# razoumov/radiativeTransfer

Measured on AMD Instinct MI355X. Metric: cell·dir·ν updates/sec per iteration, 256³ grid; achieved HBM GB/s vs peak, higher is better.
Workload: dtype f64

## Files before the change

radiativetransfer_amd/csrc/ftte_api.cpp:

```cpp
#include "ftte_context.h"

using namespace ftte;

namespace ftte {

std::string g_create_error;

int fail(ftte_ctx *c, int code, const std::string &msg)
{
    if (c) c->err = msg;
    else g_create_error = msg;
    return code;
}

int fold_status(int rc)
{
    return rc == 1 ? FTTE_ERR_PHI : rc == 2 ? FTTE_ERR_THETA : FTTE_ERR_DOMINANT_AXIS;
}

}


extern "C" {

// ... 33 lines not shown
    (void)hipSetDevice(c->device);
    if (c->stream) (void)hipStreamSynchronize(c->stream);
    for (int l = 0; l < 3; ++l) {
        if (c->kappa[l]) (void)hipFree(c->kappa[l]);
        if (c->kappa_tiled[l]) (void)hipFree(c->kappa_tiled[l]);
        if (c->emis[l]) (void)hipFree(c->emis[l]);
        for (int s = 0; s < kMaxAcc; ++s) if (c->acc[l][s]) (void)hipFree(c->acc[l][s]);
    }
    if (c->d_bdeps) (void)hipFree(c->d_bdeps);
    if (c->d_bdone) (void)hipFree(c->d_bdone);
    if (c->d_bqueue) (void)hipFree(c->d_bqueue);
    if (c->d_bsync) (void)hipFree(c->d_bsync);
    if (c->h_berror) (void)hipHostFree(c->h_berror);
    if (c->d_blayers) (void)hipFree(c->d_blayers);
    if (c->d_bgroups) (void)hipFree(c->d_bgroups);
    if (c->d_btasks) (void)hipFree(c->d_btasks);
    if (c->d_faces) (void)hipFree(c->d_faces);
    if (c->d_layers) (void)hipFree(c->d_layers);
    if (c->d_items) (void)hipFree(c->d_items);
    if (c->d_uvb) (void)hipFree(c->d_uvb);
    free_forests(c);
    free_hybrid(c);
    if (c->d_leaf_of_base) (void)hipFree(c->d_leaf_of_base);
    for (int l = 0; l < 3; ++l) if (c->base_kappa[l]) (void)hipFree(c->base_kappa[l]);
    for (int l = 0; l < 3; ++l) if (c->base_emis[l]) (void)hipFree(c->base_emis[l]);
    for (int l = 0; l < 3; ++l) {
        if (c->fine_kappa[l]) (void)hipFree(c->fine_kappa[l]);
        if (c->fine_emis[l]) (void)hipFree(c->fine_emis[l]);
        for (int a = 0; a < kMaxAcc; ++a) if (c->fine_acc[l][a]) (void)hipFree(c->fine_acc[l][a]);
    }
    if (c->amr_Iout) (void)hipFree(c->amr_Iout);
    if (c->amr_mean) (void)hipFree(c->amr_mean);
    if (c->d_amr_dirs) (void)hipFree(c->d_amr_dirs);
    if (c->d_amr_tables) (void)hipFree(c->d_amr_tables);
    if (c->amr_kappa) (void)hipFree(c->amr_kappa);
    if (c->amr_emis) (void)hipFree(c->amr_emis);
    if (c->merge_stream) (void)hipStreamDestroy(c->merge_stream);
    if (c->ev_layout_done) (void)hipEventDestroy(c->ev_layout_done);
    if (c->ev_merge_done) (void)hipEventDestroy(c->ev_merge_done);
    if (c->ev_layouts_ready) (void)hipEventDestroy(c->ev_layouts_ready);
    if (c->ev_sweep_done) (void)hipEventDestroy(c->ev_sweep_done);
    for (auto &q : c->lane_stream) (void)hipStreamDestroy(q);
    for (auto &e : c->pipe_up) (void)hipEventDestroy(e);
    for (auto &e : c->lane_done) (void)hipEventDestroy(e);
    if (c->ev_fork) (void)hipEventDestroy(c->ev_fork);
    for (auto &e : c->ev_combine) if (e) (void)hipEventDestroy(e);
    if (c->host_J_dev) (void)hipFree(c->host_J_dev);
    for (int q = 0; q < 2; ++q) {
        if (c->stage[q]) (void)hipHostFree(c->stage[q]);
        if (c->stage_ev[q]) (void)hipEventDestroy(c->stage_ev[q]);
    }
    for (auto &r : c->registered) (void)hipHostUnregister((void *)r.base);
    c->point.release();
    c->drop_chem_grid();
    if (c->chem_k) (void)hipFree(c->chem_k);
    if (c->chem_counters) (void)hipFree(c->chem_counters);
    if (c->chem_mass) (void)hipFree(c->chem_mass);
    for (auto &t : c->timing) {
        (void)hipEventDestroy(t.start); (void)hipEventDestroy(t.stop);
// ... 77 lines not shown
    if ((rc = upload(c, c->kappa[0], kappa, sizeof(double) * nnu * c->ncell))) return rc;
    c->nnu = nnu;
    c->kappa_ready[0] = true; c->kappa_ready[1] = c->kappa_ready[2] = c->kappa_ready[3] = false;
    ++c->n_kappa_sets;
    return FTTE_OK;
}

int ftte_set_opacity_device(ftte_ctx *c, int nnu, const double *kappa_dev)
{
    int rc = check_ready(c, false);
    if (rc) return rc;
    if (nnu < 1 || !kappa_dev) return fail(c, FTTE_ERR_ARG, "ftte_set_opacity_device: bad argument");
    FTTE_HIP(c, hipSetDevice(c->device));
    if ((rc = wait_sweep(c))) return rc;
    if ((rc = ensure_kappa(c, nnu))) return rc;
    const bool all_three = !c->use_forest && c->kappa[1] && c->kappa[2] && c->kappa_ready[1] && c->kappa_ready[2] && c->nnu == nnu && !c->tiled_opt;
    if (all_three) {
        if (launch_set_layouts(kappa_dev, c->kappa[0], c->kappa[1], c->kappa[2], c->n, nnu, (long)c->ncell, c->stream))
            return fail(c, FTTE_ERR_NO_DEVICE, "layout kernel launch failed");
    } else FTTE_HIP(c, hipMemcpyAsync(c->kappa[0], kappa_dev, sizeof(double) * nnu * c->ncell, hipMemcpyDeviceToDevice, c->stream));
    FTTE_HIP(c, hipStreamSynchronize(c->stream));
    c->nnu = nnu;
    c->kappa_ready[0] = true; c->kappa_ready[1] = c->kappa_ready[2] = all_three; c->kappa_ready[3] = false;
    ++c->n_kappa_sets;
    return FTTE_OK;
}

int ftte_set_species(ftte_ctx *c, int nnu, const double *HI, const double *HeI, const double *HeII, const double *beta)
{
    int rc = check_ready(c, false);
    if (rc) return rc;
    if (nnu < 1 || !HI || !HeI || !HeII || !beta) return fail(c, FTTE_ERR_ARG, "ftte_set_species: bad argument");
    FTTE_HIP(c, hipSetDevice(c->device));
    if ((rc = wait_sweep(c))) return rc;
    FTTE_HIP(c, hipStreamSynchronize(c->stream));
    if ((rc = ensure_kappa(c, nnu))) return rc;
    double *tmp = nullptr;
    const size_t nc = (size_t)c->ncell;
// ... 97 lines not shown
    } else if (!std::strcmp(key, "atomic_acc")) {
        if (value < 0 || value > 1) return fail(c, FTTE_ERR_ARG, "atomic_acc must be 0 or 1");
        c->atomic_acc = value;
    } else if (!std::strcmp(key, "ablate")) {
        if (value < 0 || value > 63) return fail(c, FTTE_ERR_ARG, "ablate is a mask of 6 bits");
        c->ablate = value;
    } else if (!std::strcmp(key, "forest_fuse")) {
        if (value < 0 || value > (1 << 24)) return fail(c, FTTE_ERR_ARG, "forest_fuse must be 0 (a launch per level) .. 16777216");
        c->forest_fuse = value;
    } else if (!std::strcmp(key, "queue_mix")) {
        if (value < 0 || value > 2) return fail(c, FTTE_ERR_ARG, "queue_mix must be 0, 1 or 2");
        c->queue_mix = value;
    } else if (!std::strcmp(key, "dataflow")) {
        if (value < 0 || value > 3) return fail(c, FTTE_ERR_ARG, "dataflow must be 0 (a launch per stage), 1 (one launch, bricks wait for each other), 2 (the same with write-through stores) or 3 (persistent workgroups, a task queue per XCD)");
        c->dataflow = value;
    } else if (!std::strcmp(key, "lanes")) {
        if (value < 1 || value > 16) return fail(c, FTTE_ERR_ARG, "lanes (streams the brick sweep spreads its frequency groups over) must be 1..16");
        c->lanes = value;
    } else if (!std::strcmp(key, "team")) {
        if (value < -1 || value > 2 || value == 1) return fail(c, FTTE_ERR_ARG, "team must be -1 (by the number of frequency groups: 2 up to four, else 0), 0 (one wavefront sweeps a group's directions in turn) or 2 (two wavefronts per brick, four rows each); 1 (a wavefront per direction) lost everywhere and is gone");
        c->team = value;
    } else if (!std::strcmp(key, "tiled")) {
        if (value < 0 || value > 2) return fail(c, FTTE_ERR_ARG, "tiled must be 0 (default), 1 (bricks: opacities and accumulators stored brick by brick where the grid is made of whole bricks: a brick's layer in one piece) or 2 (the whole brick in one piece)");
        c->tiled_opt = value;
    } else if (!std::strcmp(key, "pair_waves")) {
        if (value < 2 || value > 4) return fail(c, FTTE_ERR_ARG, "pair_waves (workgroups of two wavefronts per SIMD the pair kernel is built for) must be 2..4");
        c->pair_waves = value;
    } else if (!std::strcmp(key, "share")) {
        if (value < 0 || value > 2) return fail(c, FTTE_ERR_ARG, "share (groups sharing a J accumulator) must be 0 (none), 1 (passes of one izone) or 2 (and izone pairs)");
        c->share = value;
// ... 113 lines not shown
    if (!std::strcmp(name, "grid_builds")) return c->n_grid_builds;
    if (!std::strcmp(name, "plan_builds")) return c->n_plan_builds;
    if (!std::strcmp(name, "forest_builds")) return c->n_forest_builds;
    if (!std::strcmp(name, "hybrid_boxes")) return (c->hplan.valid && c->hplan.worthwhile) ? c->hplan.most_boxes : 0;
    if (!std::strcmp(name, "hybrid_passes")) return (c->hplan.valid && c->hplan.worthwhile) ? c->hplan.npass : 0;
    if (!std::strcmp(name, "fine_block")) return (c->hplan.valid && c->hplan.worthwhile && c->hplan.fine.active) ? c->hplan.fine.n : 0;
    if (!std::strcmp(name, "brick_form")) return c->last_brick_form;
    if (!std::strcmp(name, "brick_dataflow")) return c->last_brick_dataflow;
    if (!std::strcmp(name, "brick_chunk")) return c->bplan.valid ? c->bplan.chunk : 0;
    if (!std::strcmp(name, "brick_queue_mix")) return (c->bplan.valid && c->bplan.persistent) ? c->bplan.qmix : -1;
    if (!std::strcmp(name, "brick_groups")) return c->bplan.valid ? (long long)c->bplan.groups.size() : 0;
    if (!std::strcmp(name, "brick_accumulators")) return c->bplan.valid ? c->bplan.nacc[0] + c->bplan.nacc[1] + c->bplan.nacc[2] : 0;
    if (!std::strcmp(name, "brick_accumulators_0")) return c->bplan.valid ? c->bplan.nacc[0] : 0;
    if (!std::strcmp(name, "brick_accumulators_1")) return c->bplan.valid ? c->bplan.nacc[1] : 0;
    if (!std::strcmp(name, "brick_accumulators_2")) return c->bplan.valid ? c->bplan.nacc[2] : 0;
    return -1;
}

int ftte_launch_count(const ftte_ctx *c) { return !c ? 0 : c->multi ? multi_first(c)->timing_used : c->timing_used; }

int ftte_launch_info(ftte_ctx *c, int idx, double *ms, int64_t *updates)
{
    if (c && c->multi) return ftte_launch_info(multi_first(c), idx, ms, updates);
    if (!c || idx < 0 || idx >= c->timing_used) return FTTE_ERR_ARG;
    float t = 0.f;
    const LaunchTiming &T = c->timing[idx];
    if (T.lanes > 0) {
        float begin = 0.f, end = 0.f;
        for (int l = 0; l < T.lanes; ++l) {
            float b = 0.f, e = 0.f;
// ... 571 lines not shown
```

radiativetransfer_amd/csrc/ftte_context.h:

```cpp
#pragma once

#include <hip/hip_runtime_api.h>

#include <algorithm>
#include <cmath>
#include <cstdio>
#include <cstring>
#include <functional>
#include <string>
#include <vector>

#include <thread>

#include "../../include/ftte.h"
#include "ftte_amr.h"
#include "ftte_geometry.h"
#include "ftte_internal.h"
#include "ftte_kernels.h"
#include "ftte_point.h"


namespace ftte {


// ... 46 lines not shown
    std::vector<int32_t> deps;
    bool persistent = false;
    int qnnu = 0, nq = 0, qmix = 0;
    std::vector<uint32_t> queue;
    uint32_t qoff[kBrickQueues] = {}, qlen[kBrickQueues] = {};
    int64_t qload[kBrickQueues] = {};
    int ut = kBrickRows, uw = 0;
    int64_t uqface_off = 0;
    int nslot = 2;
    int glanes = 1, nstages = 0;
    std::vector<size_t> stage_off;
    int64_t updates = 0;
    int ntu = 0, ntv = 0, nti = 0, up = 0, vp = 0, max_dirs = 0;
    int64_t face_elems = 0, vface_off = 0, iface_off = 0;
    int nacc[3] = {0, 0, 0};
};

struct LaunchTiming {
    hipEvent_t start = nullptr, stop = nullptr;
    int64_t updates = 0;
    std::vector<hipEvent_t> first, last;
    int lanes = 0;
};


}

using namespace ftte;


// ... 74 lines not shown
        uint8_t *active = nullptr;
        std::vector<int64_t> depth_off;
        double w = 0;
    };
    std::vector<ForestDev> forests;
    std::vector<double> forest_key;
    AmrDirRec *d_amr_dirs = nullptr; size_t d_amr_dirs_cap = 0;
    int64_t *d_amr_tables = nullptr; size_t d_amr_tables_cap = 0;
    double *amr_Iout = nullptr, *amr_mean = nullptr;
    double *amr_kappa = nullptr, *amr_emis = nullptr;
    size_t amr_kappa_cap = 0, amr_emis_cap = 0;
    size_t amr_scratch_cap = 0;

    hipStream_t merge_stream = nullptr;
    hipEvent_t ev_layout_done = nullptr, ev_merge_done = nullptr, ev_layouts_ready = nullptr;
    hipEvent_t ev_sweep_done = nullptr;
    bool sweep_pending = false;

    int hybrid = 1;
    int hybrid_slots = 1;
    int use_graph = 0;
    int forest_batch = 0;
    int hybrid_lanes = 1;
    int halves = 3;
    static constexpr int kMaxPipes = 4;
    hipEvent_t ev_combine[kMaxPipes] = {nullptr, nullptr, nullptr, nullptr};
    struct HybridPlan {
        bool valid = false, worthwhile = false;
        std::vector<double> key;
        BrickPlan bricks;
// ... 188 lines not shown
```

radiativetransfer_amd/csrc/ftte_internal.h:

```cpp
#pragma once
#include <cstdint>

#include "ftte_math.h"

namespace ftte {

enum RayClass : int {
    RC_ONE = 0,
    RC_TWO_U = 1,
    RC_TWO_V = 2,
    RC_THREE_U = 3,
    RC_THREE_V = 4,
    RC_THREE_U_SWAP = 5,
    RC_THREE_V_SWAP = 6
};

struct LayerRec {
    double dpath[3];
    int32_t info;
    int32_t drift;
};
static_assert(sizeof(LayerRec) == 32, "LayerRec must be 32 bytes");

struct DirRec {
// ... 6 lines not shown
    int32_t u_lo, v_lo;
    int32_t first;
    double w;
};

struct WorkItem {
    int16_t slot;
    int16_t tu, tv;
    int16_t i_first, i_last;
    int16_t pad;
};
static_assert(sizeof(WorkItem) == 12, "WorkItem must be 12 bytes");

constexpr int kMaxSlots = 16;
constexpr int kMaxAcc = 32;

struct LaunchRec {
    DirRec dir[kMaxSlots];
    const WorkItem *items;
    const double *uvb;
    int64_t group_stride;
    int32_t n;
    int32_t nitems;
    int32_t nnu;
    int32_t emit;
    ftte_consts math;
};

constexpr int kBrickRows = 8;
constexpr int kBrickDeps = 6;
// ... 169 lines not shown
```

radiativetransfer_amd/csrc/ftte_kernels.h:

```cpp
#pragma once
#include <hip/hip_runtime_api.h>

#include "ftte_internal.h"

namespace ftte {

void set_lds_pad(int bytes);
int lds_pad();
int launch_sweep(const LaunchRec &L, int rows, int waves, int stack, int nnu, hipStream_t stream);
int launch_brick(const BrickLaunch &L, int max_dirs, int waves, hipStream_t stream, bool masked = false, int persistent = 0);
int launch_xcc_census(unsigned *mask_dev, hipStream_t stream);
int launch_brick_pair(const BrickLaunch &L, int max_dirs, int waves, hipStream_t stream);
int launch_to_layout(int layout, const double *src, double *dst, int n, int nnu, long group_stride, hipStream_t stream, bool tiled = false, int tchunk = 0);
int launch_set_layouts(const double *src, double *dst0, double *dst1, double *dst2, int n, int nnu, long group_stride, hipStream_t stream);
int launch_merge(const double *const *acc, const int *layout, int count, double *J, int n, int nnu, long group_stride,
                 bool accumulate, hipStream_t stream, const int32_t *leaf_of_base = nullptr, long j_stride = 0, bool tiled = false, int tchunk = 0);
int launch_sum_parts(const double *const *parts, int nparts, double *out, long count, hipStream_t stream);
int launch_base_cells(const double *leaf_values, const int32_t *leaf_of_base, double *base_values, long nbase, long ncell, int nnu,
                      hipStream_t stream);
int launch_amr_export(const AmrLevelRec &A, int64_t most_exports, hipStream_t stream);
int launch_amr_fine_import(const AmrLevelRec &A, int64_t most_imports, hipStream_t stream);
int launch_opacity(const double *HI, const double *HeI, const double *HeII, const double *beta, double *kappa, long ncell,
                   int nnu, hipStream_t stream);

int launch_cell_major(const double *src, double *dst, long ncell, int nnu, hipStream_t stream, const int32_t *cells = nullptr, long count = 0);
int launch_amr_level(const AmrLevelRec &A, hipStream_t stream);
int launch_amr_levels(const AmrLevelRec &A, const int64_t *tables, int ndepth, hipStream_t stream);
int launch_amr_combine(const AmrLevelRec &A, double *J, bool zero_first, hipStream_t stream);

int launch_rate_table(const FreqBin *bins, int nbins, double *tables, double *logtab, hipStream_t stream);
int launch_rate_lookup(const double *logtab, int dust, int nsample, const double *tau, double *out, hipStream_t stream);
// ... 16 lines not shown
```

radiativetransfer_amd/csrc/ftte_kernels.hip:

```cpp
#include <hip/hip_runtime.h>

#include "ftte_internal.h"
#include "ftte_kernels.h"
#include "ftte_math.h"

namespace ftte {

using gcbyte = const __attribute__((address_space(1))) char;
using gbyte = __attribute__((address_space(1))) char;
using gcdouble = const __attribute__((address_space(1))) double;
using gdouble = __attribute__((address_space(1))) double;

__device__ __forceinline__ double from_lane_below(double x)
{
    int lo = __double2loint(x), hi = __double2hiint(x);
    lo = __builtin_amdgcn_update_dpp(lo, lo, 0x138, 0xf, 0xf, false);
    hi = __builtin_amdgcn_update_dpp(hi, hi, 0x138, 0xf, 0xf, false);
    return __hiloint2double(hi, lo);
}

__device__ __forceinline__ int clampi(int x, int lo, int hi) { return x < lo ? lo : (x > hi ? hi : x); }

__device__ __forceinline__ int uniform(int x) { return __builtin_amdgcn_readfirstlane(x); }
__device__ __forceinline__ long uniform(long x)
// ... 331 lines not shown

__global__ void __launch_bounds__(256) set_layouts_kernel(const double *__restrict__ src, double *__restrict__ dst0, double *__restrict__ dst1,
                                                          double *__restrict__ dst2, int n, long group_stride)
{
    __shared__ double tile[32][33];
    const long g = blockIdx.z / n;
    const int ic = blockIdx.z % n;
    const int j0 = blockIdx.y * 32, k0 = blockIdx.x * 32;
    const int tx = threadIdx.x & 31, ty = threadIdx.x >> 5;
    const long base = g * group_stride;
    for (int r = ty; r < 32; r += 8)
        if (j0 + r < n && k0 + tx < n) {
            const double v = src[base + ((long)ic * n + j0 + r) * n + k0 + tx];
            tile[r][tx] = v;
            dst0[base + ((long)ic * n + j0 + r) * n + k0 + tx] = v;
            dst1[base + ((long)(j0 + r) * n + ic) * n + k0 + tx] = v;
        }
    __syncthreads();
    for (int r = ty; r < 32; r += 8)
        if (k0 + r < n && j0 + tx < n) dst2[base + ((long)(k0 + r) * n + ic) * n + j0 + tx] = tile[tx][r];
}

int launch_set_layouts(const double *src, double *dst0, double *dst1, double *dst2, int n, int nnu, long group_stride, hipStream_t stream)
{
    const dim3 grid((n + 31) / 32, (n + 31) / 32, n * nnu);
    hipLaunchKernelGGL(set_layouts_kernel, grid, dim3(256), 0, stream, src, dst0, dst1, dst2, n, group_stride);
    return hipGetLastError() == hipSuccess ? 0 : -2;
}

int launch_to_layout(int layout, const double *src, double *dst, int n, int nnu, long group_stride, hipStream_t stream, bool tiled, int tchunk)
{
// ... 6 lines not shown
        const dim3 grid((n + 31) / 32, (n + 31) / 32, n * nnu);
        if (tiled) hipLaunchKernelGGL(to_layout2_kernel<true>, grid, dim3(256), 0, stream, src, dst, n, group_stride, tchunk);
        else hipLaunchKernelGGL(to_layout2_kernel<false>, grid, dim3(256), 0, stream, src, dst, n, group_stride, tchunk);
    } else return -1;
    return hipGetLastError() == hipSuccess ? 0 : -2;
}

struct MergeRec {
    const double *acc[3 * kMaxAcc];
    int layout[3 * kMaxAcc];
    int count;
};

template <bool tiled>
__global__ void __launch_bounds__(256) merge_kernel(const MergeRec M, double *__restrict__ J, int n, long group_stride, int accumulate,
                                                    const int32_t *__restrict__ leaf_of_base, long j_stride, int tchunk)
{
    __shared__ double tile[32][33];
    const long g = blockIdx.z / n;
    const int ic = blockIdx.z % n;
    const int j0 = blockIdx.y * 32, k0 = blockIdx.x * 32;
    const int tx = threadIdx.x & 31, ty = threadIdx.x >> 5;
    double sum[4] = {0.0, 0.0, 0.0, 0.0};
    bool have = false;
    if (accumulate && !leaf_of_base) {
        for (int q = 0; q < 4; ++q) {
            const int jc = j0 + ty + 8 * q, kc = k0 + tx;
            if (jc < n && kc < n) sum[q] = __builtin_nontemporal_load(&J[g * group_stride + ((long)ic * n + jc) * n + kc]);
        }
        have = true;
    }
    int a0 = 0;
    while (a0 < M.count && M.layout[a0] != 2) {
        int nb = 0;
        while (nb < 8 && a0 + nb < M.count && M.layout[a0 + nb] != 2) ++nb;
        double v[8][4];
// ... 51 lines not shown
        else if (leaf_of_base[b] >= 0) {
            double *dst = &J[g * j_stride + leaf_of_base[b]];
            *dst = accumulate ? *dst + sum[q] : sum[q];
        }
    }
}

int launch_merge(const double *const *acc, const int *layout, int count, double *J, int n, int nnu, long group_stride,
                 bool accumulate, hipStream_t stream, const int32_t *leaf_of_base, long j_stride, bool tiled, int tchunk)
{
    if (count > 3 * kMaxAcc) return -1;
    MergeRec M;
    M.count = count;
    for (int a = 0; a < count; ++a) { M.acc[a] = acc[a]; M.layout[a] = layout[a]; }
    const dim3 grid((n + 31) / 32, (n + 31) / 32, n * nnu);
    if (tiled) hipLaunchKernelGGL(merge_kernel<true>, grid, dim3(256), 0, stream, M, J, n, group_stride, accumulate ? 1 : 0, leaf_of_base, j_stride, tchunk);
    else hipLaunchKernelGGL(merge_kernel<false>, grid, dim3(256), 0, stream, M, J, n, group_stride, accumulate ? 1 : 0, leaf_of_base, j_stride, tchunk);
    return hipGetLastError() == hipSuccess ? 0 : -2;
}

__device__ __forceinline__ void amr_segment(const AmrLevelRec &A, const AmrDirRec &D, int64_t begin, unsigned e, unsigned nu, unsigned nnu)
{
    const SegRec R = D.rec[begin + e];
    const int seg = R.seg, up = R.up, up2 = R.up2;
    const size_t at = (size_t)(unsigned)seg * nnu + nu;
    double I;
    if (up == -3) I = D.faces[(size_t)nu * A.face_stride + (size_t)R.at];
    else if (up < 0) I = A.uvb[nu];
    else {
        I = D.Iout[(size_t)(unsigned)up * nnu + nu];
        if (up2 >= 0) I = 0.5 * (I + D.Iout[(size_t)(unsigned)up2 * nnu + nu]);
    }
// ... 945 lines not shown
```

radiativetransfer_amd/csrc/ftte_plan.cpp:

```cpp
#include "ftte_context.h"

namespace ftte {

int plan_direction(ftte_ctx *c, int d, double phi_d, double theta_d, double w_d, int tile_rows, std::vector<ftte_pattern> &pat,
                   std::vector<int> &du_cum, std::vector<int> &dv_cum, DirPlan &D, LayerRec *layers_of_d, size_t layer_off,
                   const SubGridPlan *sub)
{
    const int n = sub ? sub->n : c->n;
    const double cell = sub ? sub->cell : c->box / (double)n;
    const long nn = (long)n * n;
    D.w = w_d;

    int rc = fold_direction(phi_d, theta_d, &D.phi, &D.theta, &D.izone);
    if (rc) {
        char buf[160];
        std::snprintf(buf, sizeof buf, "direction %d (phi=%.17g, theta=%.17g) cannot be folded: %s", d, phi_d, theta_d,
                      rc == 1 ? "phi on a quadrant boundary" : rc == 2 ? "theta outside (-pi/2,0)u(0,pi/2)"
                                                                       : "tie between dominant axes");
        return fail(c, fold_status(rc), buf);
    }
    if (sub) {
        const int src = sub->patterns(d, D.phi, D.theta, D.izone, pat.data());
        if (src) return fail(c, src, "direction " + std::to_string(d) + ": ray pattern left the unit cell (sub-layer patterns of a refined block)");
    } else if (layer_patterns(n, D.phi, D.theta, pat.data())) {
// ... 355 lines not shown
            auto &V = visits[(size_t)G.layout * kMaxAcc + G.acc];
            if (V.empty()) V.resize(nb);
            const DirPlan &D0 = P.dirs[G.dirs[0]];
            const int bu = D0.su < 0 ? P.ntu - 1 - T.tu : T.tu, bv = D0.sv < 0 ? P.ntv - 1 - T.tv : T.tv, bi = D0.si < 0 ? P.nti - 1 - ti : ti;
            V[((size_t)bi * P.ntv + bv) * P.ntu + bu].push_back({T.tu + T.tv + ti + G.offset, (int32_t)q});
        }
        for (auto &V : visits)
            for (auto &list : V) {
                std::sort(list.begin(), list.end(), [](const Visit &x, const Visit &y) { return x.launch < y.launch; });
                for (size_t k = 1; k < list.size(); ++k) P.deps[(size_t)list[k].task * kBrickDeps + 3] = list[k - 1].task;
            }
        for (size_t q = 0; q < nt; ++q)
            for (int k = 0; k < kBrickDeps; ++k)
                if (P.deps[q * kBrickDeps + k] >= (int32_t)q) return fail(c, FTTE_ERR_STATE, "brick plan: a dependency does not precede its brick");
    }
    P.persistent = false;
    if (P.dataflow && want_dataflow == 3 && !P.tasks.empty()) {
        const int nq = c->xcc_count;
        P.persistent = true; P.qnnu = nnu; P.nq = nq; P.qmix = c->queue_mix;
        std::vector<int64_t> acc_dirs(3 * (size_t)kMaxAcc, 0);
        for (const auto &G : P.groups) acc_dirs[(size_t)G.layout * kMaxAcc + G.acc] += (int64_t)G.dirs.size();
        std::vector<int> queue_of((size_t)nnu * 3 * kMaxAcc, -1);
        int64_t load[kBrickQueues] = {};
        if (nnu % nq == 0 && c->queue_mix == 0) {
            for (int nu = 0; nu < nnu; ++nu)
                for (size_t a = 0; a < acc_dirs.size(); ++a)
                    if (acc_dirs[a]) { queue_of[(size_t)nu * acc_dirs.size() + a] = nu % nq; load[nu % nq] += acc_dirs[a]; }
        } else if (c->queue_mix == 2) {
            for (int nu = 0; nu < nnu; ++nu) {
                int k = 0;
// ... 38 lines not shown
```

radiativetransfer_amd/csrc/ftte_sweeps.cpp:

```cpp
#include <cstdlib>

#include "ftte_context.h"

namespace ftte {

int ensure_kappa(ftte_ctx *c, int nnu)
{
    const size_t need = (size_t)nnu * c->ncell;
    if (c->kappa[0] && c->kappa_cap >= need) return FTTE_OK;
    for (int l = 0; l < 3; ++l) {
        if (c->kappa[l]) { FTTE_HIP(c, hipFree(c->kappa[l])); c->kappa[l] = nullptr; }
        if (c->kappa_tiled[l]) { FTTE_HIP(c, hipFree(c->kappa_tiled[l])); c->kappa_tiled[l] = nullptr; }
        if (c->emis[l]) { FTTE_HIP(c, hipFree(c->emis[l])); c->emis[l] = nullptr; }
    }
    c->emit_mode = 0;
    FTTE_HIP(c, hipMalloc((void **)&c->kappa[0], need * sizeof(double)));
    c->kappa_cap = need;
    return FTTE_OK;
}

int check_ready(ftte_ctx *c, bool need_kappa)
{
    if (c && c->multi)
        return fail(c, FTTE_ERR_UNSUPPORTED, "a multi-device context (ftte_create with ndev > 1) takes host arrays through ftte_set_grid, ftte_set_opacity, "
// ... 397 lines not shown
        c->acc_cap = per_acc;
    }
    const size_t face_need = (size_t)ndir * nnu * (size_t)P.face_elems;
    if ((rc = ensure(c, &c->d_faces, &c->d_faces_cap, face_need))) return rc;
    if (!c->merge_stream) {
        FTTE_HIP(c, hipStreamCreateWithFlags(&c->merge_stream, hipStreamNonBlocking));
        FTTE_HIP(c, hipEventCreateWithFlags(&c->ev_layout_done, hipEventDisableTiming));
        FTTE_HIP(c, hipEventCreateWithFlags(&c->ev_merge_done, hipEventDisableTiming));
        FTTE_HIP(c, hipEventCreateWithFlags(&c->ev_layouts_ready, hipEventDisableTiming));
    }
    const bool lane_ends = pipe != nullptr;
    bool lane_layout[3] = {false, false, false};
    const bool tiled = c->tiled_opt && !pipe && !c->emit_mode && n % 64 == 0 && n % kBrickRows == 0 &&
                       (c->tiled_opt == 1 || n % P.chunk == 0);
    const int tchunk = tiled && c->tiled_opt == 2 ? P.chunk : 0;
    for (int l = 0; l < 3; ++l) {
        for (int s = 0; s < P.nacc[l]; ++s)
            if (!c->acc[l][s]) FTTE_HIP(c, hipMalloc((void **)&c->acc[l][s], sizeof(double) * c->acc_cap));
        if (P.nacc[l] && tiled) {
            if (c->kappa_tiled_from[l] != c->n_kappa_sets || c->kappa_tiled_chunk[l] != tchunk) {
                if (!c->kappa_tiled[l]) FTTE_HIP(c, hipMalloc((void **)&c->kappa_tiled[l], sizeof(double) * c->kappa_cap));
                if (launch_to_layout(l, c->kappa[0], c->kappa_tiled[l], n, nnu, (long)c->ncell, stream, true, tchunk))
                    return fail(c, FTTE_ERR_NO_DEVICE, "layout kernel launch failed");
                c->kappa_tiled_from[l] = c->n_kappa_sets;
                c->kappa_tiled_chunk[l] = tchunk;
            }
        } else if (P.nacc[l] && !c->kappa_ready[l]) {
            if (!c->kappa[l]) FTTE_HIP(c, hipMalloc((void **)&c->kappa[l], sizeof(double) * c->kappa_cap));
            if (!lane_ends) {
                if (launch_to_layout(l, c->kappa[0], c->kappa[l], n, nnu, (long)c->ncell, stream))
                    return fail(c, FTTE_ERR_NO_DEVICE, "layout kernel launch failed");
                c->kappa_ready[l] = true;
            } else lane_layout[l] = true;
        }
        if (P.nacc[l] && c->emit_mode && !c->emis_ready[l]) {
            if (!c->emis[l]) FTTE_HIP(c, hipMalloc((void **)&c->emis[l], sizeof(double) * c->kappa_cap));
            if (launch_to_layout(l, c->emis[0], c->emis[l], n, nnu, (long)c->ncell, stream))
                return fail(c, FTTE_ERR_NO_DEVICE, "layout kernel launch failed");
            c->emis_ready[l] = true;
        }
    }

    if (!c->bplan_uploaded) {
        c->bgroups_sent.clear();
        if ((rc = ensure(c, &c->d_blayers, &c->d_blayers_cap, P.layers.size()))) return rc;
        if ((rc = ensure(c, &c->d_btasks, &c->d_btasks_cap, P.tasks.size()))) return rc;
        if ((rc = ensure(c, &c->d_bgroups, &c->d_bgroups_cap, P.groups.size()))) return rc;
        if (!P.layers.empty())
            FTTE_HIP(c, hipMemcpy(c->d_blayers, P.layers.data(), sizeof(LayerRec) * P.layers.size(), hipMemcpyHostToDevice));
        if (!P.tasks.empty())
            FTTE_HIP(c, hipMemcpy(c->d_btasks, P.tasks.data(), sizeof(BrickTask) * P.tasks.size(), hipMemcpyHostToDevice));
        if (P.dataflow && !P.deps.empty()) {
            if ((rc = ensure(c, &c->d_bdeps, &c->d_bdeps_cap, P.deps.size()))) return rc;
            FTTE_HIP(c, hipMemcpy(c->d_bdeps, P.deps.data(), sizeof(int32_t) * P.deps.size(), hipMemcpyHostToDevice));
        }
        c->bplan_uploaded = true;
        c->bqueue_uploaded = false;
    }
    {
        std::vector<BrickGroup> G(P.groups.size());
        std::memset(G.data(), 0, sizeof(BrickGroup) * G.size());
        for (size_t g = 0; g < P.groups.size(); ++g) {
            const BrickPlan::Group &H = P.groups[g];
            const DirPlan &D0 = P.dirs[H.dirs[0]];
            G[g].kappa = tiled ? c->kappa_tiled[H.layout] : c->kappa[H.layout];
            G[g].emis = c->emit_mode ? c->emis[H.layout] : nullptr;
            G[g].J = c->acc[H.layout][H.acc];
            G[g].org = D0.org; G[g].si = D0.si; G[g].sv = D0.sv; G[g].su = D0.su;
            if (tiled) {
                const int64_t ntu = n / 64, ntv = n / kBrickRows, piece = 64 * kBrickRows;
                G[g].sv = D0.sv > 0 ? 64 : -64;
                G[g].bu = (int32_t)(D0.su > 0 ? piece : -piece);
                G[g].bv = (int32_t)(D0.sv > 0 ? ntu * piece : -ntu * piece);
                G[g].org = (int64_t)(D0.si > 0 ? -1 : n) * n * n + (D0.sv > 0 ? 0 : (ntv - 1) * ntu * piece + (kBrickRows - 1) * 64) +
                           (D0.su > 0 ? 0 : (ntu - 1) * piece);
                if (tchunk) {
                    const int64_t nti = n / tchunk, brick = piece * tchunk;
                    G[g].si = (int32_t)(D0.si > 0 ? piece : -piece);
                    G[g].bu = (int32_t)(D0.su > 0 ? brick : -brick);
                    G[g].bv = (int32_t)(D0.sv > 0 ? ntu * brick : -ntu * brick);
                    const int64_t step_i = D0.si > 0 ? ntv * ntu * brick : -ntv * ntu * brick;
                    G[g].bi = step_i - (int64_t)tchunk * G[g].si;
                    G[g].org = (D0.si > 0 ? -piece : (nti - 1) * ntv * ntu * brick + (int64_t)tchunk * piece) +
// ... 18 lines not shown
    if (c->uvb_sent.size() != (size_t)nnu || std::memcmp(c->uvb_sent.data(), uvb, sizeof(double) * nnu) != 0) {
        FTTE_HIP(c, hipMemcpy(c->d_uvb, uvb, sizeof(double) * nnu, hipMemcpyHostToDevice));
        c->uvb_sent.assign(uvb, uvb + nnu);
    }

    const size_t nstages = (size_t)P.nstages, per_lane = nstages + 1;
    const int nulanes = P.glanes > 1 ? 1 : std::max(1, std::min(c->lanes, nnu));
    const int nlanes = nulanes * P.glanes;
    while ((int)c->lane_stream.size() < nlanes - 1) {
        hipStream_t q; hipEvent_t e;
        FTTE_HIP(c, hipStreamCreateWithFlags(&q, hipStreamNonBlocking));
        FTTE_HIP(c, hipEventCreateWithFlags(&e, hipEventDisableTiming));
        c->lane_stream.push_back(q); c->lane_done.push_back(e);
    }
    if (!c->ev_fork) FTTE_HIP(c, hipEventCreateWithFlags(&c->ev_fork, hipEventDisableTiming));
    while (c->timing.size() < 1) {
        LaunchTiming t;
        FTTE_HIP(c, hipEventCreate(&t.start));
        FTTE_HIP(c, hipEventCreate(&t.stop));
        c->timing.push_back(t);
    }
    c->timing_used = 0;

    static const ftte_consts kMath = FTTE_CONSTS_INIT;
    if (!P.groups.empty()) {
        LaunchTiming &T = c->timing[0];
        T.updates = P.updates * nnu;
        T.lanes = 0;
        if (lane_ends) {
            while ((int)T.first.size() < nlanes) {
// ... 68 lines not shown
                while (c->pipe_up.size() < (size_t)nlanes) {
                    hipEvent_t e;
                    FTTE_HIP(c, hipEventCreateWithFlags(&e, hipEventDisableTiming));
                    c->pipe_up.push_back(e);
                }
                if (lane) FTTE_HIP(c, hipStreamWaitEvent(q, c->pipe_up[(size_t)lane - 1], 0));
                if ((rc = upload_on(c, q, c->kappa[0] + slice0, pipe->kappa + slice0, slice_bytes))) return rc;
                FTTE_HIP(c, hipEventRecord(c->pipe_up[(size_t)lane], q));
            }
            if (lane_ends) {
                for (int l = 1; l < 3; ++l)
                    if (lane_layout[l] && launch_to_layout(l, c->kappa[0] + slice0, c->kappa[l] + slice0, n, nu1 - nu0, (long)c->ncell, q))
                        return fail(c, FTTE_ERR_NO_DEVICE, "layout kernel launch failed");
                FTTE_HIP(c, hipEventRecord(T.first[(size_t)lane], q));
            }
            for (size_t st = 0; st < nstages; ++st) {
                if (off[st + 1] == off[st]) continue;
                BrickLaunch L;
                std::memset(&L, 0, sizeof L);
                L.groups = c->d_bgroups;
                L.tasks = c->d_btasks + off[st];
                L.uvb = c->d_uvb;
                L.group_stride = c->ncell;
                L.face_stride = P.face_elems;
                L.vface_off = P.vface_off; L.iface_off = P.iface_off;
                L.n = n; L.ntasks = (int)(off[st + 1] - off[st]); L.nnu = nu1 - nu0; L.nu0 = nu0; L.chunk = P.chunk;
                L.up = P.up; L.vp = P.vp; L.uw = P.uw; L.ut = P.ut; L.nslot = P.nslot;
                L.emit = c->emit_mode;
                L.math = kMath;
                L.tiled = tiled ? 1 : 0;
                L.pad2_ = c->ablate;
                L.atomic_acc = c->atomic_acc;
                const int form = brick_form(c, nnu);
                c->last_brick_form = form;
                c->last_brick_dataflow = 0;
                const int lrc = form == 2 ? launch_brick_pair(L, P.max_dirs, c->pair_waves, q) : launch_brick(L, P.max_dirs, c->brick_waves, q);
                if (lrc) return fail(c, lrc == -1 ? FTTE_ERR_ARG : FTTE_ERR_NO_DEVICE, "brick kernel launch failed");
            }
            if (lane_ends) {
                FTTE_HIP(c, hipEventRecord(T.last[(size_t)lane], q));
                const double *accs[3 * kMaxAcc];
                int layouts[3 * kMaxAcc], count = 0;
                for (int l = 0; l < 3; ++l)
                    for (int s2 = 0; s2 < P.nacc[l]; ++s2) { accs[count] = c->acc[l][s2] + slice0; layouts[count++] = l; }
                if (launch_merge(accs, layouts, count, J_dev + slice0, n, nu1 - nu0, (long)c->ncell, false, q, nullptr, 0, tiled, tchunk))
                    return fail(c, FTTE_ERR_NO_DEVICE, "merge kernel launch failed");
                if (pipe && is_registered(c, pipe->J + slice0, slice_bytes))
                    FTTE_HIP(c, hipMemcpyAsync(pipe->J + slice0, J_dev + slice0, slice_bytes, hipMemcpyDeviceToHost, q));
            }
            if (lane) {
                FTTE_HIP(c, hipEventRecord(c->lane_done[(size_t)lane - 1], q));
                FTTE_HIP(c, hipStreamWaitEvent(stream, c->lane_done[(size_t)lane - 1], 0));
            }
        }
        if (pipe) {
            for (int lane = 0; lane < nlanes; ++lane) {
                const int nu0 = (int)((int64_t)nnu * lane / nulanes), nu1 = (int)((int64_t)nnu * (lane + 1) / nulanes);
                const size_t slice0 = (size_t)nu0 * c->ncell, slice_bytes = sizeof(double) * (size_t)(nu1 - nu0) * c->ncell;
                if (is_registered(c, pipe->J + slice0, slice_bytes)) continue;
                hipStream_t q = lane == 0 ? stream : c->lane_stream[(size_t)lane - 1];
                if ((rc = download_on(c, q, pipe->J + slice0, J_dev + slice0, slice_bytes))) return rc;
            }
            c->kappa_ready[0] = true;
            ++c->n_kappa_sets;
        }
        if (lane_ends) {
            for (int l = 1; l < 3; ++l) if (lane_layout[l]) c->kappa_ready[l] = true;
            T.lanes = nlanes;
        }
        FTTE_HIP(c, hipEventRecord(T.stop, stream));
        c->timing_used = 1;
    }
    if (!lane_ends || P.groups.empty()) {
        const double *accs[3 * kMaxAcc];
        int layouts[3 * kMaxAcc], count = 0;
        for (int l = 0; l < 3; ++l)
            for (int s = 0; s < P.nacc[l]; ++s) { accs[count] = c->acc[l][s]; layouts[count++] = l; }
        if (count) {
            if (launch_merge(accs, layouts, count, J_dev, n, nnu, (long)c->ncell, false, stream, nullptr, 0, tiled, tchunk))
                return fail(c, FTTE_ERR_NO_DEVICE, "merge kernel launch failed");
        } else FTTE_HIP(c, hipMemsetAsync(J_dev, 0, sizeof(double) * (size_t)nnu * c->ncell, stream));
    }
    return mark_sweep(c, stream);
}


int tile_sweep(ftte_ctx *c, int ndir, const double *phi, const double *theta, const double *w, const double *uvb, double *J_dev,
               hipStream_t stream)
{
    int rc;
    const int n = c->n, nnu = c->nnu;
    const size_t per_acc = (size_t)nnu * c->ncell;
// ... 134 lines not shown
```

Baseline: 379.6 billion.

## Overlap J merge with brick sweep stages and reuse layout-0 kappa for layout 1

The plan now records the last sweep stage that touches each 32³ block. After selected stages it records events, and a side merge stream merges the finished blocks into J while later brick stages still run. This hides most of the final merge pass behind the sweep. Separately, layout-1 groups now read layout-0 kappa through remapped strides, so the layout-1 transpose copy is skipped. In exchange the merge kernels share bandwidth with the sweep, and each merge point adds events and launches.

```diff
diff --git a/radiativetransfer_amd/csrc/ftte_api.cpp b/radiativetransfer_amd/csrc/ftte_api.cpp
--- a/radiativetransfer_amd/csrc/ftte_api.cpp
+++ b/radiativetransfer_amd/csrc/ftte_api.cpp
@@ -71,6 +71,7 @@
     if (c->h_berror) (void)hipHostFree(c->h_berror);
     if (c->d_blayers) (void)hipFree(c->d_blayers);
     if (c->d_bgroups) (void)hipFree(c->d_bgroups);
+    if (c->d_mblocks) (void)hipFree(c->d_mblocks);
     if (c->d_btasks) (void)hipFree(c->d_btasks);
     if (c->d_faces) (void)hipFree(c->d_faces);
     if (c->d_layers) (void)hipFree(c->d_layers);
@@ -100,6 +101,7 @@
     for (auto &q : c->lane_stream) (void)hipStreamDestroy(q);
     for (auto &e : c->pipe_up) (void)hipEventDestroy(e);
     for (auto &e : c->lane_done) (void)hipEventDestroy(e);
+    for (auto &e : c->ev_merge_point) (void)hipEventDestroy(e);
     if (c->ev_fork) (void)hipEventDestroy(c->ev_fork);
     for (auto &e : c->ev_combine) if (e) (void)hipEventDestroy(e);
     if (c->host_J_dev) (void)hipFree(c->host_J_dev);
@@ -207,14 +209,15 @@
     FTTE_HIP(c, hipSetDevice(c->device));
     if ((rc = wait_sweep(c))) return rc;
     if ((rc = ensure_kappa(c, nnu))) return rc;
-    const bool all_three = !c->use_forest && c->kappa[1] && c->kappa[2] && c->kappa_ready[1] && c->kappa_ready[2] && c->nnu == nnu && !c->tiled_opt;
-    if (all_three) {
-        if (launch_set_layouts(kappa_dev, c->kappa[0], c->kappa[1], c->kappa[2], c->n, nnu, (long)c->ncell, c->stream))
+    const bool same = !c->use_forest && c->nnu == nnu && !c->tiled_opt;
+    const bool with2 = same && c->kappa[2] && c->kappa_ready[2], with1 = with2 && c->kappa[1] && c->kappa_ready[1];
+    if (with2) {
+        if (launch_set_layouts(kappa_dev, c->kappa[0], with1 ? c->kappa[1] : nullptr, c->kappa[2], c->n, nnu, (long)c->ncell, c->stream))
             return fail(c, FTTE_ERR_NO_DEVICE, "layout kernel launch failed");
     } else FTTE_HIP(c, hipMemcpyAsync(c->kappa[0], kappa_dev, sizeof(double) * nnu * c->ncell, hipMemcpyDeviceToDevice, c->stream));
     FTTE_HIP(c, hipStreamSynchronize(c->stream));
     c->nnu = nnu;
-    c->kappa_ready[0] = true; c->kappa_ready[1] = c->kappa_ready[2] = all_three; c->kappa_ready[3] = false;
+    c->kappa_ready[0] = true; c->kappa_ready[1] = with1; c->kappa_ready[2] = with2; c->kappa_ready[3] = false;
     ++c->n_kappa_sets;
     return FTTE_OK;
 }
@@ -342,6 +345,9 @@
     } else if (!std::strcmp(key, "dataflow")) {
         if (value < 0 || value > 3) return fail(c, FTTE_ERR_ARG, "dataflow must be 0 (a launch per stage), 1 (one launch, bricks wait for each other), 2 (the same with write-through stores) or 3 (persistent workgroups, a task queue per XCD)");
         c->dataflow = value;
+    } else if (!std::strcmp(key, "merge_overlap")) {
+        if (value != 0 && value != 1) return fail(c, FTTE_ERR_ARG, "merge_overlap must be 0 (the brick sweep merges J after its last stage) or 1 (block by block as the stages finish them)");
+        c->merge_overlap = value;
     } else if (!std::strcmp(key, "lanes")) {
         if (value < 1 || value > 16) return fail(c, FTTE_ERR_ARG, "lanes (streams the brick sweep spreads its frequency groups over) must be 1..16");
         c->lanes = value;
@@ -485,6 +491,15 @@
     if (!std::strcmp(name, "brick_accumulators_0")) return c->bplan.valid ? c->bplan.nacc[0] : 0;
     if (!std::strcmp(name, "brick_accumulators_1")) return c->bplan.valid ? c->bplan.nacc[1] : 0;
     if (!std::strcmp(name, "brick_accumulators_2")) return c->bplan.valid ? c->bplan.nacc[2] : 0;
+    if (!std::strcmp(name, "brick_stages")) return c->bplan.valid ? c->bplan.nstages : 0;
+    if (!std::strcmp(name, "merge_points")) return c->bplan.valid ? (long long)c->bplan.merge_stage.size() : 0;
+    if (!std::strcmp(name, "merge_blocks")) return c->bplan.valid ? (long long)c->bplan.merge_blocks.size() : 0;
+    if (!std::strncmp(name, "merge_stage_", 12) || !std::strncmp(name, "merge_final_", 12)) {
+        char *end = nullptr;
+        const long k = std::strtol(name + 12, &end, 10);
+        if (!c->bplan.valid || end == name + 12 || *end || k < 0 || k >= (long)c->bplan.merge_stage.size()) return -1;
+        return name[6] == 's' ? c->bplan.merge_stage[(size_t)k] : (long long)c->bplan.merge_off[(size_t)k + 1];
+    }
     return -1;
 }
 
diff --git a/radiativetransfer_amd/csrc/ftte_context.h b/radiativetransfer_amd/csrc/ftte_context.h
--- a/radiativetransfer_amd/csrc/ftte_context.h
+++ b/radiativetransfer_amd/csrc/ftte_context.h
@@ -84,6 +84,10 @@
     int ntu = 0, ntv = 0, nti = 0, up = 0, vp = 0, max_dirs = 0;
     int64_t face_elems = 0, vface_off = 0, iface_off = 0;
     int nacc[3] = {0, 0, 0};
+    int nmb = 0;
+    std::vector<int32_t> merge_blocks;
+    std::vector<int> merge_stage;
+    std::vector<size_t> merge_off;
 };
 
 struct LaunchTiming {
@@ -188,6 +192,9 @@
 
     hipStream_t merge_stream = nullptr;
     hipEvent_t ev_layout_done = nullptr, ev_merge_done = nullptr, ev_layouts_ready = nullptr;
+    int merge_overlap = 1;
+    std::vector<hipEvent_t> ev_merge_point;
+    int32_t *d_mblocks = nullptr; size_t d_mblocks_cap = 0;
     hipEvent_t ev_sweep_done = nullptr;
     bool sweep_pending = false;
 
diff --git a/radiativetransfer_amd/csrc/ftte_internal.h b/radiativetransfer_amd/csrc/ftte_internal.h
--- a/radiativetransfer_amd/csrc/ftte_internal.h
+++ b/radiativetransfer_amd/csrc/ftte_internal.h
@@ -44,6 +44,7 @@
 
 constexpr int kMaxSlots = 16;
 constexpr int kMaxAcc = 32;
+constexpr int kMergeBlock = 32;
 
 struct LaunchRec {
     DirRec dir[kMaxSlots];
diff --git a/radiativetransfer_amd/csrc/ftte_kernels.h b/radiativetransfer_amd/csrc/ftte_kernels.h
--- a/radiativetransfer_amd/csrc/ftte_kernels.h
+++ b/radiativetransfer_amd/csrc/ftte_kernels.h
@@ -15,6 +15,8 @@
 int launch_set_layouts(const double *src, double *dst0, double *dst1, double *dst2, int n, int nnu, long group_stride, hipStream_t stream);
 int launch_merge(const double *const *acc, const int *layout, int count, double *J, int n, int nnu, long group_stride,
                  bool accumulate, hipStream_t stream, const int32_t *leaf_of_base = nullptr, long j_stride = 0, bool tiled = false, int tchunk = 0);
+int launch_merge_blocks(const double *const *acc, const int *layout, int count, double *J, int n, int nnu, long group_stride,
+                        const int32_t *blocks, int nblocks, int nmb, hipStream_t stream, bool tiled = false, int tchunk = 0);
 int launch_sum_parts(const double *const *parts, int nparts, double *out, long count, hipStream_t stream);
 int launch_base_cells(const double *leaf_values, const int32_t *leaf_of_base, double *base_values, long nbase, long ncell, int nnu,
                       hipStream_t stream);
diff --git a/radiativetransfer_amd/csrc/ftte_kernels.hip b/radiativetransfer_amd/csrc/ftte_kernels.hip
--- a/radiativetransfer_amd/csrc/ftte_kernels.hip
+++ b/radiativetransfer_amd/csrc/ftte_kernels.hip
@@ -369,7 +369,7 @@
             const double v = src[base + ((long)ic * n + j0 + r) * n + k0 + tx];
             tile[r][tx] = v;
             dst0[base + ((long)ic * n + j0 + r) * n + k0 + tx] = v;
-            dst1[base + ((long)(j0 + r) * n + ic) * n + k0 + tx] = v;
+            if (dst1) dst1[base + ((long)(j0 + r) * n + ic) * n + k0 + tx] = v;
         }
     __syncthreads();
     for (int r = ty; r < 32; r += 8)
@@ -406,12 +406,25 @@
 
 template <bool tiled>
 __global__ void __launch_bounds__(256) merge_kernel(const MergeRec M, double *__restrict__ J, int n, long group_stride, int accumulate,
-                                                    const int32_t *__restrict__ leaf_of_base, long j_stride, int tchunk)
-{
+                                                    const int32_t *__restrict__ leaf_of_base, long j_stride, int tchunk,
+                                                    const int32_t *__restrict__ blocks, int nmb)
+{
+    static_assert(kMergeBlock == 32, "a merge block is one tile per ic plane");
     __shared__ double tile[32][33];
-    const long g = blockIdx.z / n;
-    const int ic = blockIdx.z % n;
-    const int j0 = blockIdx.y * 32, k0 = blockIdx.x * 32;
+    long g;
+    int ic, j0, k0;
+    if (blocks) {
+        const int b = blocks[blockIdx.x];
+        const int bi = b / (nmb * nmb), bj = (b / nmb) % nmb, bk = b % nmb;
+        g = blockIdx.z;
+        ic = bi * kMergeBlock + (int)blockIdx.y;
+        j0 = bj * kMergeBlock; k0 = bk * kMergeBlock;
+        if (ic >= n) return;
+    } else {
+        g = blockIdx.z / n;
+        ic = blockIdx.z % n;
+        j0 = blockIdx.y * 32; k0 = blockIdx.x * 32;
+    }
     const int tx = threadIdx.x & 31, ty = threadIdx.x >> 5;
     double sum[4] = {0.0, 0.0, 0.0, 0.0};
     bool have = false;
@@ -493,8 +506,22 @@
     M.count = count;
     for (int a = 0; a < count; ++a) { M.acc[a] = acc[a]; M.layout[a] = layout[a]; }
     const dim3 grid((n + 31) / 32, (n + 31) / 32, n * nnu);
-    if (tiled) hipLaunchKernelGGL(merge_kernel<true>, grid, dim3(256), 0, stream, M, J, n, group_stride, accumulate ? 1 : 0, leaf_of_base, j_stride, tchunk);
-    else hipLaunchKernelGGL(merge_kernel<false>, grid, dim3(256), 0, stream, M, J, n, group_stride, accumulate ? 1 : 0, leaf_of_base, j_stride, tchunk);
+    if (tiled) hipLaunchKernelGGL(merge_kernel<true>, grid, dim3(256), 0, stream, M, J, n, group_stride, accumulate ? 1 : 0, leaf_of_base, j_stride, tchunk, nullptr, 0);
+    else hipLaunchKernelGGL(merge_kernel<false>, grid, dim3(256), 0, stream, M, J, n, group_stride, accumulate ? 1 : 0, leaf_of_base, j_stride, tchunk, nullptr, 0);
+    return hipGetLastError() == hipSuccess ? 0 : -2;
+}
+
+int launch_merge_blocks(const double *const *acc, const int *layout, int count, double *J, int n, int nnu, long group_stride,
+                        const int32_t *blocks, int nblocks, int nmb, hipStream_t stream, bool tiled, int tchunk)
+{
+    if (count > 3 * kMaxAcc || nmb != (n + kMergeBlock - 1) / kMergeBlock) return -1;
+    if (nblocks == 0 || nnu == 0) return 0;
+    MergeRec M;
+    M.count = count;
+    for (int a = 0; a < count; ++a) { M.acc[a] = acc[a]; M.layout[a] = layout[a]; }
+    const dim3 grid(nblocks, kMergeBlock, nnu);
+    if (tiled) hipLaunchKernelGGL(merge_kernel<true>, grid, dim3(256), 0, stream, M, J, n, group_stride, 0, nullptr, 0l, tchunk, blocks, nmb);
+    else hipLaunchKernelGGL(merge_kernel<false>, grid, dim3(256), 0, stream, M, J, n, group_stride, 0, nullptr, 0l, tchunk, blocks, nmb);
     return hipGetLastError() == hipSuccess ? 0 : -2;
 }
 
diff --git a/radiativetransfer_amd/csrc/ftte_plan.cpp b/radiativetransfer_amd/csrc/ftte_plan.cpp
--- a/radiativetransfer_amd/csrc/ftte_plan.cpp
+++ b/radiativetransfer_amd/csrc/ftte_plan.cpp
@@ -393,6 +393,53 @@
             for (int k = 0; k < kBrickDeps; ++k)
                 if (P.deps[q * kBrickDeps + k] >= (int32_t)q) return fail(c, FTTE_ERR_STATE, "brick plan: a dependency does not precede its brick");
     }
+    P.nmb = 0; P.merge_blocks.clear(); P.merge_stage.clear(); P.merge_off.clear();
+    if (!P.dataflow && P.glanes == 1 && !P.tasks.empty()) {
+        const int nmb = (n + kMergeBlock - 1) / kMergeBlock;
+        const size_t nblk = (size_t)nmb * nmb * nmb;
+        P.nmb = nmb;
+        std::vector<int> last(nblk, nstages - 1);
+        std::vector<char> seen(nblk, 0);
+        for (int st = 0; st < nstages; ++st)
+            for (size_t q = P.stage_off[(size_t)st]; q < P.stage_off[(size_t)st + 1]; ++q) {
+                const BrickTask &T = P.tasks[q];
+                const BrickPlan::Group &G = P.groups[(size_t)T.group];
+                const DirPlan &D0 = P.dirs[G.dirs[0]];
+                const int march_c = G.layout, fast_c = march_c == 2 ? 1 : 2, mid_c = march_c == 0 ? 1 : 0;
+                int lo[3], hi[3];
+                auto span = [&](int axis, int first, int len, bool mirror) {
+                    const int a = first, b = std::min(first + len, n) - 1;
+                    lo[axis] = (mirror ? n - 1 - b : a) / kMergeBlock;
+                    hi[axis] = (mirror ? n - 1 - a : b) / kMergeBlock;
+                };
+                span(march_c, chunk * (T.ti & (kBrickAccumulate - 1)), chunk, D0.si < 0);
+                span(mid_c, kBrickRows * T.tv, kBrickRows, D0.sv < 0);
+                span(fast_c, 64 * T.tu, 64, D0.su < 0);
+                for (int bi = lo[0]; bi <= hi[0]; ++bi)
+                    for (int bj = lo[1]; bj <= hi[1]; ++bj)
+                        for (int bk = lo[2]; bk <= hi[2]; ++bk) {
+                            const size_t b = ((size_t)bi * nmb + bj) * nmb + bk;
+                            last[b] = seen[b] ? std::max(last[b], st) : st;
+                            seen[b] = 1;
+                        }
+            }
+        std::vector<int32_t> order(nblk);
+        for (size_t b = 0; b < nblk; ++b) order[b] = (int32_t)b;
+        std::stable_sort(order.begin(), order.end(), [&](int32_t x, int32_t y) { return last[(size_t)x] < last[(size_t)y]; });
+        static const double kFrac[] = {4. / 8, 6. / 8, 7. / 8, 15. / 16, 31. / 32, 1.};
+        P.merge_off.push_back(0);
+        for (double f : kFrac) {
+            const size_t want = std::min(nblk, std::max<size_t>(1, (size_t)std::ceil(f * (double)nblk)));
+            const int st = f >= 1. ? nstages - 1 : last[(size_t)order[want - 1]];
+            if (!P.merge_stage.empty() && st <= P.merge_stage.back()) continue;
+            size_t end = P.merge_off.back();
+            while (end < nblk && last[(size_t)order[end]] <= st) ++end;
+            if (end == P.merge_off.back() && st != nstages - 1) continue;
+            P.merge_stage.push_back(st);
+            P.merge_off.push_back(end);
+        }
+        P.merge_blocks = std::move(order);
+    }
     P.persistent = false;
     if (P.dataflow && want_dataflow == 3 && !P.tasks.empty()) {
         const int nq = c->xcc_count;
diff --git a/radiativetransfer_amd/csrc/ftte_sweeps.cpp b/radiativetransfer_amd/csrc/ftte_sweeps.cpp
--- a/radiativetransfer_amd/csrc/ftte_sweeps.cpp
+++ b/radiativetransfer_amd/csrc/ftte_sweeps.cpp
@@ -435,6 +435,7 @@
     const bool tiled = c->tiled_opt && !pipe && !c->emit_mode && n % 64 == 0 && n % kBrickRows == 0 &&
                        (c->tiled_opt == 1 || n % P.chunk == 0);
     const int tchunk = tiled && c->tiled_opt == 2 ? P.chunk : 0;
+    auto frame = [tiled](int l) { return l == 1 && !tiled ? 0 : l; };
     for (int l = 0; l < 3; ++l) {
         for (int s = 0; s < P.nacc[l]; ++s)
             if (!c->acc[l][s]) FTTE_HIP(c, hipMalloc((void **)&c->acc[l][s], sizeof(double) * c->acc_cap));
@@ -446,7 +447,7 @@
                 c->kappa_tiled_from[l] = c->n_kappa_sets;
                 c->kappa_tiled_chunk[l] = tchunk;
             }
-        } else if (P.nacc[l] && !c->kappa_ready[l]) {
+        } else if (P.nacc[l] && frame(l) == l && !c->kappa_ready[l]) {
             if (!c->kappa[l]) FTTE_HIP(c, hipMalloc((void **)&c->kappa[l], sizeof(double) * c->kappa_cap));
             if (!lane_ends) {
                 if (launch_to_layout(l, c->kappa[0], c->kappa[l], n, nnu, (long)c->ncell, stream))
@@ -454,7 +455,7 @@
                 c->kappa_ready[l] = true;
             } else lane_layout[l] = true;
         }
-        if (P.nacc[l] && c->emit_mode && !c->emis_ready[l]) {
+        if (P.nacc[l] && frame(l) == l && c->emit_mode && !c->emis_ready[l]) {
             if (!c->emis[l]) FTTE_HIP(c, hipMalloc((void **)&c->emis[l], sizeof(double) * c->kappa_cap));
             if (launch_to_layout(l, c->emis[0], c->emis[l], n, nnu, (long)c->ncell, stream))
                 return fail(c, FTTE_ERR_NO_DEVICE, "layout kernel launch failed");
@@ -475,6 +476,10 @@
             if ((rc = ensure(c, &c->d_bdeps, &c->d_bdeps_cap, P.deps.size()))) return rc;
             FTTE_HIP(c, hipMemcpy(c->d_bdeps, P.deps.data(), sizeof(int32_t) * P.deps.size(), hipMemcpyHostToDevice));
         }
+        if (!P.merge_blocks.empty()) {
+            if ((rc = ensure(c, &c->d_mblocks, &c->d_mblocks_cap, P.merge_blocks.size()))) return rc;
+            FTTE_HIP(c, hipMemcpy(c->d_mblocks, P.merge_blocks.data(), sizeof(int32_t) * P.merge_blocks.size(), hipMemcpyHostToDevice));
+        }
         c->bplan_uploaded = true;
         c->bqueue_uploaded = false;
     }
@@ -484,10 +489,16 @@
         for (size_t g = 0; g < P.groups.size(); ++g) {
             const BrickPlan::Group &H = P.groups[g];
             const DirPlan &D0 = P.dirs[H.dirs[0]];
-            G[g].kappa = tiled ? c->kappa_tiled[H.layout] : c->kappa[H.layout];
-            G[g].emis = c->emit_mode ? c->emis[H.layout] : nullptr;
+            G[g].kappa = tiled ? c->kappa_tiled[H.layout] : c->kappa[frame(H.layout)];
+            G[g].emis = c->emit_mode ? c->emis[frame(H.layout)] : nullptr;
             G[g].J = c->acc[H.layout][H.acc];
             G[g].org = D0.org; G[g].si = D0.si; G[g].sv = D0.sv; G[g].su = D0.su;
+            if (frame(H.layout) != H.layout) {
+                const int64_t nn = (int64_t)n * n;
+                G[g].si = D0.si > 0 ? n : -n;
+                G[g].sv = (int32_t)(D0.sv > 0 ? nn : -nn);
+                G[g].org = -1 + (D0.sv > 0 ? -nn : n * nn) + (D0.si > 0 ? -(int64_t)n : nn);
+            }
             if (tiled) {
                 const int64_t ntu = n / 64, ntv = n / kBrickRows, piece = 64 * kBrickRows;
                 G[g].sv = D0.sv > 0 ? 64 : -64;
@@ -536,6 +547,13 @@
         c->lane_stream.push_back(q); c->lane_done.push_back(e);
     }
     if (!c->ev_fork) FTTE_HIP(c, hipEventCreateWithFlags(&c->ev_fork, hipEventDisableTiming));
+    const bool overlap = c->merge_overlap && !lane_ends && !P.dataflow && P.glanes == 1 && !P.groups.empty() && !P.merge_stage.empty();
+    const size_t npoints = overlap ? P.merge_stage.size() : 0;
+    while (c->ev_merge_point.size() < (size_t)nlanes * npoints) {
+        hipEvent_t e;
+        FTTE_HIP(c, hipEventCreateWithFlags(&e, hipEventDisableTiming));
+        c->ev_merge_point.push_back(e);
+    }
     while (c->timing.size() < 1) {
         LaunchTiming t;
         FTTE_HIP(c, hipEventCreate(&t.start));
@@ -634,8 +652,18 @@
                         return fail(c, FTTE_ERR_NO_DEVICE, "layout kernel launch failed");
                 FTTE_HIP(c, hipEventRecord(T.first[(size_t)lane], q));
             }
-            for (size_t st = 0; st < nstages; ++st) {
-                if (off[st + 1] == off[st]) continue;
+            for (size_t st = 0, mp = 0; st < nstages; ++st) {
+                auto merge_point = [&]() -> int {
+                    if (overlap && mp < npoints && (size_t)P.merge_stage[mp] == st) {
+                        FTTE_HIP(c, hipEventRecord(c->ev_merge_point[(size_t)lane * npoints + mp], q));
+                        ++mp;
+                    }
+                    return FTTE_OK;
+                };
+                if (off[st + 1] == off[st]) {
+                    if ((rc = merge_point())) return rc;
+                    continue;
+                }
                 BrickLaunch L;
                 std::memset(&L, 0, sizeof L);
                 L.groups = c->d_bgroups;
@@ -656,13 +684,14 @@
                 c->last_brick_dataflow = 0;
                 const int lrc = form == 2 ? launch_brick_pair(L, P.max_dirs, c->pair_waves, q) : launch_brick(L, P.max_dirs, c->brick_waves, q);
                 if (lrc) return fail(c, lrc == -1 ? FTTE_ERR_ARG : FTTE_ERR_NO_DEVICE, "brick kernel launch failed");
+                if ((rc = merge_point())) return rc;
             }
             if (lane_ends) {
                 FTTE_HIP(c, hipEventRecord(T.last[(size_t)lane], q));
                 const double *accs[3 * kMaxAcc];
                 int layouts[3 * kMaxAcc], count = 0;
                 for (int l = 0; l < 3; ++l)
-                    for (int s2 = 0; s2 < P.nacc[l]; ++s2) { accs[count] = c->acc[l][s2] + slice0; layouts[count++] = l; }
+                    for (int s2 = 0; s2 < P.nacc[l]; ++s2) { accs[count] = c->acc[l][s2] + slice0; layouts[count++] = frame(l); }
                 if (launch_merge(accs, layouts, count, J_dev + slice0, n, nu1 - nu0, (long)c->ncell, false, q, nullptr, 0, tiled, tchunk))
                     return fail(c, FTTE_ERR_NO_DEVICE, "merge kernel launch failed");
                 if (pipe && is_registered(c, pipe->J + slice0, slice_bytes))
@@ -691,11 +720,29 @@
         FTTE_HIP(c, hipEventRecord(T.stop, stream));
         c->timing_used = 1;
     }
-    if (!lane_ends || P.groups.empty()) {
+    if (overlap) {
         const double *accs[3 * kMaxAcc];
         int layouts[3 * kMaxAcc], count = 0;
         for (int l = 0; l < 3; ++l)
-            for (int s = 0; s < P.nacc[l]; ++s) { accs[count] = c->acc[l][s]; layouts[count++] = l; }
+            for (int s = 0; s < P.nacc[l]; ++s) { accs[count] = c->acc[l][s]; layouts[count++] = frame(l); }
+        for (size_t mp = 0; mp < npoints; ++mp)
+            for (int lane = 0; lane < nlanes; ++lane) {
+                const int nu0 = (int)((int64_t)nnu * lane / nulanes), nu1 = (int)((int64_t)nnu * (lane + 1) / nulanes);
+                const size_t slice0 = (size_t)nu0 * c->ncell;
+                const double *lane_accs[3 * kMaxAcc];
+                for (int a = 0; a < count; ++a) lane_accs[a] = accs[a] + slice0;
+                FTTE_HIP(c, hipStreamWaitEvent(c->merge_stream, c->ev_merge_point[(size_t)lane * npoints + mp], 0));
+                if (launch_merge_blocks(lane_accs, layouts, count, J_dev + slice0, n, nu1 - nu0, (long)c->ncell, c->d_mblocks + P.merge_off[mp],
+                                        (int)(P.merge_off[mp + 1] - P.merge_off[mp]), P.nmb, c->merge_stream, tiled, tchunk))
+                    return fail(c, FTTE_ERR_NO_DEVICE, "merge kernel launch failed");
+            }
+        FTTE_HIP(c, hipEventRecord(c->ev_merge_done, c->merge_stream));
+        FTTE_HIP(c, hipStreamWaitEvent(stream, c->ev_merge_done, 0));
+    } else if (!lane_ends || P.groups.empty()) {
+        const double *accs[3 * kMaxAcc];
+        int layouts[3 * kMaxAcc], count = 0;
+        for (int l = 0; l < 3; ++l)
+            for (int s = 0; s < P.nacc[l]; ++s) { accs[count] = c->acc[l][s]; layouts[count++] = frame(l); }
         if (count) {
             if (launch_merge(accs, layouts, count, J_dev, n, nnu, (long)c->ncell, false, stream, nullptr, 0, tiled, tchunk))
                 return fail(c, FTTE_ERR_NO_DEVICE, "merge kernel launch failed");
```

Result: faster. 392.7 billion, median of 6 (+3.5%).
